# tum-vision/LDSO

Hardware: AMD Instinct MI355X
Metric: GN iters/sec + Mresiduals/sec, 7-KF/2000-pt window (higher is better)
Workload: dtype f32; 1 GPU; C3: 7 KF x 2000 pt x 8 px, 640x480, R=12000, forced GN iterations, synthetic rank-6 marginalisation prior H_M/b_M; arithmetic=f32 residuals / Jacobians / accumulators as the reference, f64 stitch and solve, parallelism=1 GPU

## Files before the change

ldso_amd/csrc/ba_reduce.hip:

```cpp
#include <hip/hip_runtime.h>
#include "ba_host.h"

#include "ba_reduce_body.h"

__global__ __launch_bounds__(256) void k_reduce(BaPtrs B, BaDims D, ResSet S, ChunkStarts chunkStart, int hasL, int GSP, int atomicMode,
                                                int hasPrior, float calibPrior, double l1, double il, int itCheck) {
    static_assert(sizeof(BaPtrs) + sizeof(BaDims) + sizeof(ResSet) + sizeof(ChunkStarts) >= 8 * 64 - 60, "k_reduce: ld_touch_kernarg<8> must stay inside the arguments");
    ld_touch_kernarg<8>();
    reduce_body(B, D, S, chunkStart, hasL, GSP, atomicMode, hasPrior, calibPrior, l1, il, itCheck, (int) blockIdx.x);
}

static __device__ __forceinline__ int g_col(int i, int FS) { return (i < 4) ? (8 * FS + i) : (i - 4); }

static __device__ __forceinline__ double sum_f(const double *PC, int F, int base, int stride, int off, double init = 0.0) {
    double q[LD_MAXF];
#pragma unroll
    for (int x = 0; x < LD_MAXF; x++) q[x] = (x < F) ? PC[(size_t) (base + x * stride) * LD_PAIRC + off] : 0.0;
    double v = init;
#pragma unroll
    for (int x = 0; x < LD_MAXF; x++) if (x < F) v += q[x];
    return v;
}
static __device__ __forceinline__ double sum_pairs(const double *PC, int F, int off) {
    double v = 0;
    for (int p0 = 0; p0 < F * F; p0 += 16) {
        double q[16];
#pragma unroll
        for (int x = 0; x < 16; x++) q[x] = (p0 + x < F * F) ? PC[(size_t) (p0 + x) * LD_PAIRC + off] : 0.0;
#pragma unroll
        for (int x = 0; x < 16; x++) if (p0 + x < F * F) v += q[x];
    }
    return v;
}

static __device__ __forceinline__ double top_entry(const double *PC, int F, int i, int j) {
    if (j < 0) {
        if (i < 4) return sum_pairs(PC, F, 288 + i);
        int f = (i - 4) >> 3, a = (i - 4) & 7;
        double v = sum_f(PC, F, f * F, 1, 272 + a);
        return sum_f(PC, F, f, F, 280 + a, v);
    }
    if (i < 4 && j < 4) return sum_pairs(PC, F, 256 + i * 4 + j);
    if (i < 4 || j < 4) {
        int fi = (i < 4) ? j : i, c = (i < 4) ? i : j;
        int f = (fi - 4) >> 3, a = (fi - 4) & 7;
        double v = sum_f(PC, F, f * F, 1, 192 + a * 4 + c);
        return sum_f(PC, F, f, F, 224 + a * 4 + c, v);
    }
    int f = (i - 4) >> 3, a = (i - 4) & 7, g = (j - 4) >> 3, c = (j - 4) & 7;
    if (f == g) {
        double v = sum_f(PC, F, f * F, 1, a * 8 + c);
        return sum_f(PC, F, f, F, 64 + a * 8 + c, v);
    }
    if (f < g) return PC[(size_t) (f * F + g) * LD_PAIRC + 128 + a * 8 + c] + PC[(size_t) (g * F + f) * LD_PAIRC + 128 + c * 8 + a];
    return PC[(size_t) (g * F + f) * LD_PAIRC + 128 + c * 8 + a] + PC[(size_t) (f * F + g) * LD_PAIRC + 128 + a * 8 + c];
}

__global__ __launch_bounds__(256) void k_gather(BaPtrs B, BaDims D, ResSet S, int hasL, int hasPrior, int GSP, double lambdaIn, int solverMode,
                                                float calibPrior, int mode, double *rbuf) {
    const int F = D.F, n = D.n, FS = D.FS;
    const int N = n * n + n;
    const int e = blockIdx.x * blockDim.x + threadIdx.x;
    double lambda = lambdaIn;
    if (solverMode & LDSO_SOLVER_USE_GN) lambda = 0;
    if (solverMode & LDSO_SOLVER_FIX_LAMBDA) lambda = 1e-5;
    const size_t blk = (size_t) n * n + n;
    double *HA = B.sys, *bA = HA + n * n, *HL = bA + n, *bL = HL + n * n, *Hsc = bL + n, *bsc = Hsc + n * n, *HF = bsc + n, *bF = HF + n * n;
    if (mode == 1 && e >= N && e < N + D.P) {
        int i = e - N;
        double v = 0.0;
        if (i >= D.pBegin && i < D.pEnd) { float c = S.candE[i]; if (c >= 0.0f) v = (double) c + 1.0; }
        rbuf[3 * blk + 8 + i] = v;
    }
    if (e >= N) return;
    const int i = (e < n * n) ? e / n : (e - n * n), j = (e < n * n) ? e % n : -1;
    double prH = 0, prb = 0;
    if (j < 0) prb = (i < 4) ? (double) calibPrior * (double) B.calib->cDeltaF[i] : B.frames[(i - 4) >> 3].prior[(i - 4) & 7] * B.frames[(i - 4) >> 3].delta_prior[(i - 4) & 7];
    else if (i == j) prH = (i < 4) ? (double) calibPrior : B.frames[(i - 4) >> 3].prior[(i - 4) & 7];

    double vA, vL, vS;
    if (mode == 2) {
        vA = rbuf[e]; vL = rbuf[blk + e]; vS = rbuf[2 * blk + e];
    } else {
        vA = top_entry(B.pairC, F, i, j);
        vL = hasL ? top_entry(B.pairC + (size_t) F * F * LD_PAIRC, F, i, j) : 0.0;
        int ci = g_col(i, FS), cj = (j >= 0) ? g_col(j, FS) : (8 * FS + 4);
        int r = min(ci, cj), c = max(ci, cj);
        size_t off = (r / 16 == c / 16) ? ((size_t) ci * GSP + cj) : ((size_t) r * GSP + c);
        float q[LD_SC_SPLITS];
#pragma unroll
        for (int sp = 0; sp < LD_SC_SPLITS; sp++) q[sp] = B.scPart[(size_t) sp * GSP * GSP + off];
        vS = 0;
#pragma unroll
        for (int sp = 0; sp < LD_SC_SPLITS; sp++) vS += (double) q[sp];
    }
    if (mode == 1) { rbuf[e] = vA; rbuf[blk + e] = vL; rbuf[2 * blk + e] = vS; return; }
    if (j >= 0) { HA[e] = vA; HL[e] = vL + prH; Hsc[e] = vS; }
    else { bA[i] = vA; bL[i] = vL + prb; bsc[i] = vS; }
    if (j >= 0) {
        double v = (vL + prH) + (hasPrior ? B.HM[e] : 0.0) + vA;
        if (i == j) v *= (1 + lambda);
        v -= vS * (double) (1.0f / (1 + lambda));
        HF[e] = v;
    } else {
        double s = 0;
        if (hasPrior) {
            s = B.bM[i];
            for (int jj = 0; jj < n; jj++) {
                double dj = (jj < 4) ? (double) B.calib->cDeltaF[jj] : B.frames[(jj - 4) >> 3].delta[(jj - 4) & 7];
                s += B.HM[(size_t) i * n + jj] * dj;
            }
        }
        bF[i] = (vL + prb) + s + vA - vS;
    }
}

hipError_t ba_launch_gather(const BaPtrs &B, const BaDims &D, const ResSet &S, bool hasL, bool hasPrior, int GSP, double lambda,
                            const ldso_settings_t &St, int mode, double *rbuf, hipStream_t st) {
    int N = D.n * D.n + D.n + (mode == 1 ? D.P : 0);
    hipLaunchKernelGGL(k_gather, dim3((N + 255) / 256), dim3(256), 0, st, B, D, S, hasL ? 1 : 0, hasPrior ? 1 : 0, GSP, lambda, St.solverMode,
                       St.initialCalibHessian, mode, rbuf);
    return hipGetLastError();
}

hipError_t ba_launch_reduce(const BaPtrs &B, const BaDims &D, const ResSet &S, const ChunkStarts &chunkStart, bool hasL, int GSP, int atomicMode, bool hasPrior,
                            float calibPrior, double l1, double il, int itCheck, hipStream_t st) {
    const int nb = atomicMode ? reduce_grid(D.F, hasL, D.ks, GSP).total : reduce_pairs(D.F, hasL) + LD_SC_SPLITS;
    const size_t lds = atomicMode ? reduce_atomic_lds_bytes() : (size_t) (SC_SLAB * GSP) * sizeof(float);
    return launch_lds(k_reduce, dim3(nb), dim3(256), lds, st, B, D, S, chunkStart, hasL ? 1 : 0, GSP, atomicMode, hasPrior ? 1 : 0, calibPrior, l1, il, itCheck);
}

__global__ __launch_bounds__(256) void k_marg_update(BaPtrs B, BaDims D, double w) {
    const int n = D.n, e = blockIdx.x * blockDim.x + threadIdx.x;
    const double *HA = B.sys, *bA = HA + n * n, *Hsc = bA + n + (size_t) n * n + n, *bsc = Hsc + n * n;
    if (e < n * n) B.HM[e] += (HA[e] - Hsc[e]) * w;
    else if (e < n * n + n) B.bM[e - n * n] += (bA[e - n * n] - bsc[e - n * n]) * w;
}

hipError_t ba_launch_marg_update(const BaPtrs &B, const BaDims &D, double w, hipStream_t st) {
    const int N = D.n * D.n + D.n;
    hipLaunchKernelGGL(k_marg_update, dim3((N + 255) / 256), dim3(256), 0, st, B, D, w);
    return hipGetLastError();
}

__global__ __launch_bounds__(256) void k_reduce_batch_marg(const BatchItem *__restrict__ items, const MargWin *__restrict__ mw, int nWin) {
    int w = 0;
    for (int i = 1; i < nWin; i++) if ((int) blockIdx.x >= mw[i].redBlock0) w = i;
    const MargWin m = mw[w];
    if (!m.active) return;
    const BatchItem &it = items[w];
    reduce_body(it.B, it.D, it.set[1], it.cs, 0, it.GSP, 0, 0, 0.0f, 1.0, 1.0, -1, (int) blockIdx.x - m.redBlock0);
}

hipError_t ba_launch_reduce_batch_marg(const BatchItem *d_items, const MargWin *d_mw, int nWin, int totalBlocks, int maxGSP, hipStream_t st) {
    if (totalBlocks <= 0) return hipSuccess;
    return launch_lds(k_reduce_batch_marg, dim3(totalBlocks), dim3(256), (size_t) (SC_SLAB * maxGSP) * sizeof(float), st, d_items, d_mw, nWin);
}

__global__ __launch_bounds__(256) void k_marg_gather_update_batch(const BatchItem *__restrict__ items, const MargWin *__restrict__ mw, double w, double *__restrict__ out) {
    const MargWin m = mw[blockIdx.y];
    if (!m.active) return;
    const BatchItem &it = items[blockIdx.y];
    const int F = it.D.F, n = it.D.n, FS = it.D.FS, GSP = it.GSP;
    const int e = blockIdx.x * blockDim.x + threadIdx.x;
    if (e >= n * n + n) return;
    const int i = (e < n * n) ? e / n : (e - n * n), j = (e < n * n) ? e % n : -1;
    const double vA = top_entry(it.B.pairC, F, i, j);
    const int ci = g_col(i, FS), cj = (j >= 0) ? g_col(j, FS) : (8 * FS + 4);
    const int r = min(ci, cj), c = max(ci, cj);
    const size_t off = (r / 16 == c / 16) ? ((size_t) ci * GSP + cj) : ((size_t) r * GSP + c);
    float q[LD_SC_SPLITS];
#pragma unroll
    for (int sp = 0; sp < LD_SC_SPLITS; sp++) q[sp] = it.B.scPart[(size_t) sp * GSP * GSP + off];
    double vS = 0;
#pragma unroll
    for (int sp = 0; sp < LD_SC_SPLITS; sp++) vS += (double) q[sp];
    double *dst = (j >= 0) ? it.B.HM + e : it.B.bM + i;
    double v = it.hasPrior ? *dst : 0.0;
    v += (vA - vS) * w;
    *dst = v;
    out[(size_t) m.outOff + e] = v;
}

hipError_t ba_launch_marg_gather_update_batch(const BatchItem *d_items, const MargWin *d_mw, int nWin, int maxN, double w, double *d_out, hipStream_t st) {
    const int N = maxN * maxN + maxN;
    hipLaunchKernelGGL(k_marg_gather_update_batch, dim3((N + 255) / 256, nWin), dim3(256), 0, st, d_items, d_mw, w, d_out);
    return hipGetLastError();
}

static __device__ __forceinline__ void marg_frame_body(BaPtrs B, BaDims D, int idx, double *W, double *outH, double *outb) {
    const int tid = threadIdx.x, n = D.n, nd = n - 8;
    double *Hs = W, *bs = W + (size_t) n * n;
    __shared__ double sSV[8 * LD_MAXF + 4], sHpi[64], sLU[64], sBLI[(8 * LD_MAXF + 4) * 8];
    __shared__ int sPiv[8];
    auto perm = [&](int i) { const int io = 4 + 8 * idx; return (i < io) ? i : (i < nd) ? i + 8 : io + (i - nd); };
    const DevFrame &fh = B.frames[idx];
    for (int e = tid; e < n * n; e += 256) {
        const int i = e / n, j = e % n;
        double v = B.HM[(size_t) perm(i) * n + perm(j)];
        if (i == j && i >= nd) v += fh.prior[i - nd];
        Hs[e] = v;
    }
    for (int i = tid; i < n; i += 256) bs[i] = B.bM[perm(i)] + ((i >= nd) ? fh.prior[i - nd] * fh.delta_prior[i - nd] : 0.0);
    __syncthreads();
    for (int i = tid; i < n; i += 256) sSV[i] = sqrt(fabs(Hs[(size_t) i * n + i]) + 10.0);
    __syncthreads();
    for (int e = tid; e < n * n; e += 256) { const int i = e / n, j = e % n; Hs[e] = (1.0 / sSV[i]) * Hs[e] * (1.0 / sSV[j]); }
    for (int i = tid; i < n; i += 256) bs[i] = (1.0 / sSV[i]) * bs[i];
    __syncthreads();
    if (tid < 64) { const int r = tid >> 3, c = tid & 7; const double v = Hs[(size_t) (nd + r) * n + nd + c]; sLU[tid] = 0.5 * (v + v); }
    __syncthreads();
    if (tid == 0) {
        for (int k = 0; k < 8; k++) {
            int p = k; double best = fabs(sLU[k * 8 + k]);
            for (int i = k + 1; i < 8; i++) if (fabs(sLU[i * 8 + k]) > best) { best = fabs(sLU[i * 8 + k]); p = i; }
            sPiv[k] = p;
            if (p != k) for (int j = 0; j < 8; j++) { double t = sLU[k * 8 + j]; sLU[k * 8 + j] = sLU[p * 8 + j]; sLU[p * 8 + j] = t; }
            for (int i = k + 1; i < 8; i++) {
                sLU[i * 8 + k] /= sLU[k * 8 + k];
                for (int j = k + 1; j < 8; j++) sLU[i * 8 + j] -= sLU[i * 8 + k] * sLU[k * 8 + j];
            }
        }
    }
    __syncthreads();
    if (tid < 8) {
        double x[8];
        for (int i = 0; i < 8; i++) x[i] = (i == tid) ? 1.0 : 0.0;
        for (int k = 0; k < 8; k++) { const int p = sPiv[k]; if (p != k) { double t = x[k]; x[k] = x[p]; x[p] = t; } }
        for (int i = 0; i < 8; i++) for (int j = 0; j < i; j++) x[i] -= sLU[i * 8 + j] * x[j];
        for (int i = 7; i >= 0; i--) { for (int j = i + 1; j < 8; j++) x[i] -= sLU[i * 8 + j] * x[j]; x[i] /= sLU[i * 8 + i]; }
        for (int i = 0; i < 8; i++) sHpi[i * 8 + tid] = x[i];
    }
    __syncthreads();
    if (tid < 64) sHpi[tid] = 0.5 * (sHpi[tid] + sHpi[tid]);
    __syncthreads();
    for (int e = tid; e < nd * 8; e += 256) {
        const int i = e >> 3, c = e & 7;
        double s_ = 0;
        for (int k = 0; k < 8; k++) s_ += Hs[(size_t) (nd + k) * n + i] * sHpi[k * 8 + c];
        sBLI[e] = s_;
    }
    __syncthreads();
    for (int e = tid; e < nd * (nd + 1); e += 256) {
        const int i = e / (nd + 1), j = e % (nd + 1);
        const double *bl = sBLI + i * 8;
        double s_ = 0;
        if (j < nd) { for (int k = 0; k < 8; k++) s_ += bl[k] * Hs[(size_t) (nd + k) * n + j]; Hs[(size_t) i * n + j] -= s_; }
        else { for (int k = 0; k < 8; k++) s_ += bl[k] * bs[nd + k]; bs[i] -= s_; }
    }
    __syncthreads();
    for (int e = tid; e < nd * nd; e += 256) {
        const int i = e / nd, j = e % nd;
        outH[e] = 0.5 * (sSV[i] * Hs[(size_t) i * n + j] * sSV[j] + sSV[j] * Hs[(size_t) j * n + i] * sSV[i]);
    }
    for (int i = tid; i < nd; i += 256) outb[i] = sSV[i] * bs[i];
}

__global__ __launch_bounds__(256) void k_marg_frame(BaPtrs B, BaDims D, int idx, double *W, double *outH, double *outb) {
    marg_frame_body(B, D, idx, W, outH, outb);
}

__global__ __launch_bounds__(256) void k_marg_frame_batch(const BatchItem *__restrict__ items, const MargWin *__restrict__ mw, double *__restrict__ out) {
    const MargWin m = mw[blockIdx.x];
    if (!m.active) return;
    const BatchItem &it = items[blockIdx.x];
    const int n = it.D.n, nd = n - 8;
    if (!it.hasPrior) {
        for (int e = threadIdx.x; e < n * n; e += 256) it.B.HM[e] = 0.0;
        for (int e = threadIdx.x; e < n; e += 256) it.B.bM[e] = 0.0;
        __syncthreads();
    }
    double *oH = out + m.outOff;
    marg_frame_body(it.B, it.D, m.frameIdx, it.B.sys, oH, oH + (size_t) nd * nd);
}

hipError_t ba_launch_marg_frame_batch(const BatchItem *d_items, int nWin, const MargWin *d_mw, double *d_out, hipStream_t st) {
    hipLaunchKernelGGL(k_marg_frame_batch, dim3(nWin), dim3(256), 0, st, d_items, d_mw, d_out);
    return hipGetLastError();
}

hipError_t ba_launch_marg_frame(const BaPtrs &B, const BaDims &D, int idx, double *work, double *outH, double *outb, hipStream_t st) {
    hipLaunchKernelGGL(k_marg_frame, dim3(1), dim3(256), 0, st, B, D, idx, work, outH, outb);
    return hipGetLastError();
}

__global__ __launch_bounds__(256) void k_acc_init(BaPtrs B, BaDims D, GnInit gi) {
    const int n = D.n, e = blockIdx.x * blockDim.x + threadIdx.x;
    if (e >= n * n + n) return;
    double v = 0.0;
    if (e < n * n && gi.enable == 1) {
        const int i = e / n, j = e % n;
        if (j <= i) {
            if (gi.hasPrior) v = B.HM[e];
            if (i == j) v += (i < 4) ? (double) gi.calibPrior : B.frames[(i - 4) >> 3].prior[(i - 4) & 7];
        }
    }
    B.acc[e] = v;
}

hipError_t ba_launch_acc_init(const BaPtrs &B, const BaDims &D, const GnInit &gi, hipStream_t st) {
    const int N = D.n * D.n + D.n;
    hipLaunchKernelGGL(k_acc_init, dim3((N + 255) / 256), dim3(256), 0, st, B, D, gi);
    return hipGetLastError();
}
```

ldso_amd/csrc/ba_reduce_body.h:

```cpp
#pragma once
#include <hip/hip_runtime.h>
#include "ba_dev.h"

typedef float f32x4 __attribute__((ext_vector_type(4)));
#define SC_SLAB 128
#define PA_SLICES 2
#define PA_UNROLL 24
#define SCT_KS LD_SCT_KS
#define SCT_SLAB 512
#define SC_MAXT 12

__host__ __device__ constexpr int tri13r(int r, int c) { return r * 13 - (r * (r - 1)) / 2 + (c - r); }
__host__ __device__ constexpr size_t reduce_atomic_lds_bytes() { return (size_t) (2 * SCT_SLAB * 16 + SCT_SLAB) * sizeof(float); }

static __device__ __forceinline__ void acc_add(double *p, double v) { __hip_atomic_fetch_add(p, v, __ATOMIC_RELAXED, __HIP_MEMORY_SCOPE_AGENT); }

template <int NT, int W> static __device__ __forceinline__ void schur_wave(const float *sG, int GSP, int cnt, int wcol, int li, int lk, f32x4 *acc);

static __device__ __forceinline__ void reduce_body(const BaPtrs &B, const BaDims &D, const ResSet &S, const ChunkStarts &chunkStart, int hasL, int GSP, int atomicMode,
                                   int hasPrior, float calibPrior, double l1, double il, int itCheck, const int bid) {
    if (LD_ITER_SKIPPED(B, itCheck)) return;
    const int F = D.F, FS = D.FS;
    const int nPairBlocks = reduce_pairs(F, hasL);
    const int tid = threadIdx.x;
    __shared__ double sA[13 * 13];
    __shared__ double sT[2][64];
    const long long t0_ = wall_clock64();
#define RSTAMP(i) do { if (LD_STAMP_ON && tid == 0) B.energyLog[(i)] = (double) (wall_clock64() - t0_); } while (0)

    if (bid < nPairBlocks) {
        const int which = bid / (F * F);
        const int pair = bid % (F * F);
        const int h = pair / F, t = pair % F;
        const float *part = which ? S.topL : S.topA;
        const int c0 = chunkStart.v[h], c1 = chunkStart.v[h + 1];
        if (bid == 0 && c1 > c0) RSTAMP(22);
        __shared__ double sAH[64], sAT[64];
        __shared__ double sPart[PA_SLICES][LD_TOPN];
        if (tid >= 128 && tid < 192) { sAH[tid - 128] = B.adHost[(size_t) (h + t * F) * 64 + (tid - 128)]; }
        if (tid >= 192) { sAT[tid - 192] = B.adTarget[(size_t) (h + t * F) * 64 + (tid - 192)]; }
        const int slice = tid / LD_TOPN, ent = tid % LD_TOPN;
        if (slice < PA_SLICES) {
            double a = 0;
            for (int cb = c0 + slice; cb < c1; cb += PA_SLICES * PA_UNROLL) {
                float q[PA_UNROLL];
#pragma unroll
                for (int u = 0; u < PA_UNROLL; u++) {
                    const int c = cb + u * PA_SLICES, cc = max(min(c, c1 - 1), 0);
                    const float v = part[((unsigned) cc * (unsigned) FS + (unsigned) t) * LD_TOPN + (unsigned) ent];
                    q[u] = (c < c1) ? v : 0.0f;
                }
#pragma unroll
                for (int u = 0; u < PA_UNROLL; u++) a += (double) q[u];
            }
            sPart[slice][ent] = a;
            if (bid == 0 && a != 12345.678) RSTAMP(23);
        }
        __syncthreads();
        if (bid == 0) RSTAMP(20);
        if (tid < LD_TOPN) {
            double a = sPart[0][tid];
#pragma unroll
            for (int sl = 1; sl < PA_SLICES; sl++) a += sPart[sl][tid];
            int r = 0, rem = tid;
            while (rem >= 13 - r) { rem -= 13 - r; r++; }
            int cidx = r + rem;
            sA[r * 13 + cidx] = a;
            sA[cidx * 13 + r] = a;
        }
        __syncthreads();
        double *out = B.pairC + ((size_t) which * F * F + pair) * LD_PAIRC;
        const double *AH = sAH, *AT = sAT;
        if (tid < 64) {
            int i = tid >> 3, j = tid & 7;
            double th = 0, tt = 0;
            for (int m = 0; m < 8; m++) { th += AH[i * 8 + m] * sA[(4 + m) * 13 + 4 + j]; tt += AT[i * 8 + m] * sA[(4 + m) * 13 + 4 + j]; }
            sT[0][tid] = th; sT[1][tid] = tt;
        }
        __syncthreads();
        const int n = D.n;
        double *accT = B.acc, *accb = B.acc + (size_t) n * n;
        const int rh = 4 + 8 * h, rt = 4 + 8 * t;
        if (tid < 64) {
            int i = tid >> 3, j = tid & 7;
            double hh = 0, tt = 0, ht = 0;
            for (int m = 0; m < 8; m++) { hh += sT[0][i * 8 + m] * AH[j * 8 + m]; tt += sT[1][i * 8 + m] * AT[j * 8 + m]; ht += sT[0][i * 8 + m] * AT[j * 8 + m]; }
            if (!atomicMode) { out[tid] = hh; out[64 + tid] = tt; out[128 + tid] = ht; }
            else {
                if (i >= j) { const double dsc = (i == j) ? l1 : 1.0; acc_add(&accT[(size_t) (rh + i) * n + rh + j], hh * dsc); acc_add(&accT[(size_t) (rt + i) * n + rt + j], tt * dsc); }
                if (h > t) acc_add(&accT[(size_t) (rh + i) * n + rt + j], ht);
                else if (h < t) acc_add(&accT[(size_t) (rt + j) * n + rh + i], ht);
            }
        } else if (tid < 64 + 32) {
            int e = tid - 64, i = e >> 2, c = e & 3;
            double hc = 0, tc = 0;
            for (int m = 0; m < 8; m++) { hc += AH[i * 8 + m] * sA[(4 + m) * 13 + c]; tc += AT[i * 8 + m] * sA[(4 + m) * 13 + c]; }
            if (!atomicMode) { out[192 + e] = hc; out[224 + e] = tc; }
            else { acc_add(&accT[(size_t) (rh + i) * n + c], hc); acc_add(&accT[(size_t) (rt + i) * n + c], tc); }
        } else if (tid < 96 + 16) {
            int e = tid - 96;
            if (!atomicMode) out[256 + e] = sA[(e >> 2) * 13 + (e & 3)];
            else if ((e >> 2) >= (e & 3)) acc_add(&accT[(size_t) (e >> 2) * n + (e & 3)], sA[(e >> 2) * 13 + (e & 3)] * (((e >> 2) == (e & 3)) ? l1 : 1.0));
        } else if (tid < 112 + 8) {
            int i = tid - 112;
            double bh = 0, bt = 0;
            for (int m = 0; m < 8; m++) { bh += AH[i * 8 + m] * sA[(4 + m) * 13 + 12]; bt += AT[i * 8 + m] * sA[(4 + m) * 13 + 12]; }
            if (!atomicMode) { out[272 + i] = bh; out[280 + i] = bt; }
            else { acc_add(&accb[rh + i], bh); acc_add(&accb[rt + i], bt); }
        } else if (tid < 120 + 4) {
            int i = tid - 120;
            if (!atomicMode) out[288 + i] = sA[i * 13 + 12];
            else acc_add(&accb[i], sA[i * 13 + 12]);
        }
        if (bid == 0) RSTAMP(21);
        return;
    }

    const int nSplitBase = nPairBlocks;
    const int KS = D.ks;
    if (atomicMode && bid < nSplitBase + reduce_tiles(KS, GSP)) {
        extern __shared__ __attribute__((aligned(16))) float sT_[];
        float *sAc = sT_, *sBc = sAc + SCT_SLAB * 16, *sWc = sBc + SCT_SLAB * 16;
        const int bb = bid - nSplitBase, tile = bb / KS, ks = bb % KS;
        const int nT = GSP / 16, GS = D.GS, n = D.n;
        int ti = 0, rem = tile;
        while (rem >= nT - ti) { rem -= nT - ti; ti++; }
        const int tj = ti + rem;
        const int P0 = D.pBegin, Pn = D.pEnd - D.pBegin, per = ((Pn + KS - 1) / KS + 3) & ~3;
        const int pa = P0 + ks * per, pb = min(P0 + Pn, pa + per);
        const int wave = tid >> 6, lane = tid & 63, li = lane & 15, lk = lane >> 4;
        const int wcol = 8 * FS + 5;
        f32x4 acc = (f32x4){0.f, 0.f, 0.f, 0.f}, acc2 = acc;
        for (int base = pa; base < pb; base += SCT_SLAB) {
            const int cnt = min(SCT_SLAB, pb - base), rows = (cnt + 3) & ~3;
            __syncthreads();
            {
                float4 q[16];
                float wq[2];
#pragma unroll
                for (int u = 0; u < 16; u++) {
                    const int e = tid + u * 256, r = e >> 3, half = (e >> 2) & 1, c4 = e & 3;
                    const int col = (half ? tj : ti) * 16 + c4 * 4;
                    const float4 v = *(const float4 *) (S.G + (unsigned) ((base + min(r, cnt - 1)) * GS + min(col, GS - 4)));
                    const bool in = r < cnt && col < GS;
                    q[u] = make_float4(in ? v.x : 0.f, in ? v.y : 0.f, in ? v.z : 0.f, in ? v.w : 0.f);
                }
#pragma unroll
                for (int u = 0; u < 2; u++) { const int r = tid + u * 256; const float v = S.G[(unsigned) ((base + min(r, cnt - 1)) * GS + wcol)]; wq[u] = (r < cnt) ? v : 0.f; }
#pragma unroll
                for (int u = 0; u < 16; u++) {
                    const int e = tid + u * 256, r = e >> 3, half = (e >> 2) & 1, c4 = e & 3;
                    if (r < rows) *(float4 *) ((half ? sBc : sAc) + r * 16 + c4 * 4) = q[u];
                }
#pragma unroll
                for (int u = 0; u < 2; u++) { const int r = tid + u * 256; if (r < rows) sWc[r] = wq[u]; }
            }
            __syncthreads();
            if (bb == 0) RSTAMP(25);
#pragma unroll 4
            for (int k0 = wave * 4; k0 < rows; k0 += 32) {
                const int k1 = k0 + 16;
                const float a0 = sAc[(k0 + lk) * 16 + li] * sWc[k0 + lk], b0 = sBc[(k0 + lk) * 16 + li];
                const bool in1 = k1 < rows;
                const int k1c = in1 ? k1 : k0;
                const float a1 = in1 ? sAc[(k1c + lk) * 16 + li] * sWc[k1c + lk] : 0.f, b1 = sBc[(k1c + lk) * 16 + li];
                acc = __builtin_amdgcn_mfma_f32_16x16x4f32(a0, b0, acc, 0, 0, 0);
                acc2 = __builtin_amdgcn_mfma_f32_16x16x4f32(a1, b1, acc2, 0, 0, 0);
            }
        }
        __syncthreads();
        if (bb == 0) RSTAMP(26);
        float *sR = sT_;
#pragma unroll
        for (int r = 0; r < 4; r++) sR[wave * 256 + (lk * 4 + r) * 16 + li] = acc[r] + acc2[r];
        __syncthreads();
        {
            const float v = ((sR[tid] + sR[256 + tid]) + sR[512 + tid]) + sR[768 + tid];
            const int rr = ti * 16 + (tid >> 4), cc = tj * 16 + (tid & 15);
            const int F8 = 8 * D.F, FS8 = 8 * FS;
            const int I = (rr < F8) ? 4 + rr : (rr >= FS8 && rr < FS8 + 4) ? rr - FS8 : (rr == FS8 + 4) ? n : -1;
            const int J = (cc < F8) ? 4 + cc : (cc >= FS8 && cc < FS8 + 4) ? cc - FS8 : (cc == FS8 + 4) ? n : -1;
            const bool use = !(ti == tj && rr > cc) && I >= 0 && J >= 0 && I != n;
            if (use) {
                if (J == n) acc_add(&B.acc[(size_t) n * n + I], -(double) v);
                else acc_add(&B.acc[(size_t) max(I, J) * n + min(I, J)], -(double) v * il);
            }
        }
        if (bb == 0) RSTAMP(27);
        return;
    }
    if (atomicMode == 2) return;
    if (atomicMode) {
        const int n = D.n;
        __shared__ double sDelta[8 * LD_MAXF + 4];
        if (tid < n) sDelta[tid] = (tid < 4) ? (double) B.calib->cDeltaF[tid] : B.frames[(tid - 4) >> 3].delta[(tid - 4) & 7];
        double prb = 0, prH = 0, bm = 0;
        if (tid < n) {
            if (tid < 4) { prH = (double) calibPrior; prb = (double) calibPrior * (double) B.calib->cDeltaF[tid]; }
            else { const DevFrame &f = B.frames[(tid - 4) >> 3]; prH = f.prior[(tid - 4) & 7]; prb = prH * f.delta_prior[(tid - 4) & 7]; }
            if (hasPrior) bm = B.bM[tid];
        }
        const int rowT = tid >> 2, quarter = tid & 3;
        constexpr int QW = 16;
        double hq[QW];
        const int per = (n + 3) >> 2, j0 = quarter * per;
        const bool rowOn = hasPrior && rowT < n && 4 * n <= 256;
#pragma unroll
        for (int u = 0; u < QW; u++) hq[u] = (rowOn && u < per && j0 + u < n) ? B.HM[(size_t) rowT * n + j0 + u] : 0.0;
        __syncthreads();
        double part = 0;
#pragma unroll
        for (int u = 0; u < QW; u++) if (u < per && j0 + u < n) part += hq[u] * sDelta[j0 + u];
        part += __shfl_xor(part, 1, 64); part += __shfl_xor(part, 2, 64);
        __shared__ double sHd[8 * LD_MAXF + 4];
        if (quarter == 0 && rowT < n) sHd[rowT] = part;
        __syncthreads();
        if (tid < n) {
            double s_ = 0;
            if (hasPrior) {
                s_ = bm;
                if (4 * n <= 256) s_ += sHd[tid];
                else for (int j0_ = 0; j0_ < n; j0_ += 16) {
                    double q[16];
#pragma unroll
                    for (int u = 0; u < 16; u++) q[u] = (j0_ + u < n) ? B.HM[(size_t) tid * n + j0_ + u] : 0.0;
#pragma unroll
                    for (int u = 0; u < 16; u++) if (j0_ + u < n) s_ += q[u] * sDelta[j0_ + u];
                }
            }
            acc_add(&B.acc[(size_t) n * n + tid], prb + s_);
            const double dterm = prH + (hasPrior ? B.HM[(size_t) tid * n + tid] : 0.0);
            acc_add(&B.acc[(size_t) tid * n + tid], dterm * (l1 - 1.0));
        }
        RSTAMP(28);
        return;
    }

    extern __shared__ __attribute__((aligned(16))) float sG[];
    const int sp = bid - nSplitBase;
    const int wave = tid >> 6, lane = tid & 63;
    const int nT = GSP / 16;
    const int P0 = D.pBegin, Pn = D.pEnd - D.pBegin;
    const int per = (Pn + LD_SC_SPLITS - 1) / LD_SC_SPLITS;
    const int pa = P0 + sp * per, pb = min(P0 + Pn, pa + per);
    const int GS = D.GS;
    const int li = lane & 15, lk = lane >> 4;
    float *Mout = B.scPart + (size_t) sp * GSP * GSP;
    f32x4 acc[SC_MAXT];
#pragma unroll
    for (int q = 0; q < SC_MAXT; q++) acc[q] = (f32x4){0.f, 0.f, 0.f, 0.f};
    for (int base = pa; base < pb; base += SC_SLAB) {
        const int cnt = min(SC_SLAB, pb - base);
        __syncthreads();
        {
            const int g4 = GS >> 2, p4 = GSP >> 2;
            const int rows = (cnt + 3) & ~3;
            for (int e0 = tid; e0 < rows * p4; e0 += 256 * 8) {
                float4 q[8];
#pragma unroll
                for (int u = 0; u < 8; u++) {
                    const int e = e0 + u * 256, r = e / p4, c = e % p4;
                    q[u] = make_float4(0.f, 0.f, 0.f, 0.f);
                    if (e < rows * p4 && r < cnt && c < g4) q[u] = ((const float4 *) (S.G + (size_t) (base + r) * GS))[c];
                }
#pragma unroll
                for (int u = 0; u < 8; u++) { const int e = e0 + u * 256; if (e < rows * p4) ((float4 *) sG)[e] = q[u]; }
            }
        }
        __syncthreads();
        if (sp == 0) RSTAMP(22);
        const int wcol = 8 * FS + 5;
        if (nT == 5) {
            if (wave == 0) schur_wave<5, 0>(sG, GSP, cnt, wcol, li, lk, acc); else if (wave == 1) schur_wave<5, 1>(sG, GSP, cnt, wcol, li, lk, acc);
            else if (wave == 2) schur_wave<5, 2>(sG, GSP, cnt, wcol, li, lk, acc); else schur_wave<5, 3>(sG, GSP, cnt, wcol, li, lk, acc);
        } else {
            if (wave == 0) schur_wave<9, 0>(sG, GSP, cnt, wcol, li, lk, acc); else if (wave == 1) schur_wave<9, 1>(sG, GSP, cnt, wcol, li, lk, acc);
            else if (wave == 2) schur_wave<9, 2>(sG, GSP, cnt, wcol, li, lk, acc); else schur_wave<9, 3>(sG, GSP, cnt, wcol, li, lk, acc);
        }
    }
    if (sp == 0) RSTAMP(23);
    {
        const int n = D.n, F8 = 8 * D.F, FS8 = 8 * FS;
        double *accS = B.acc, *accSb = accS + (size_t) n * n;
        const double *unused_ = nullptr; (void) unused_;
        for (int pass = 0; pass < 1; pass++) {
            int tileIdx = 0;
            for (int ti = 0; ti < nT; ti++)
                for (int tj = ti; tj < nT; tj++, tileIdx++) {
                    if ((tileIdx & 3) != wave) continue;
                    const int q = tileIdx >> 2;
                    f32x4 a4 = acc[0];
#pragma unroll
                    for (int u = 1; u < SC_MAXT; u++) if (u == q) a4 = acc[u];
#pragma unroll
                    for (int r = 0; r < 4; r++) {
                        const int rr = ti * 16 + lk * 4 + r, cc = tj * 16 + li;
                        if (!atomicMode) { Mout[(size_t) rr * GSP + cc] = a4[r]; continue; }
                        if (ti == tj && rr > cc) continue;
                        const int I = (rr < F8) ? 4 + rr : (rr >= FS8 && rr < FS8 + 4) ? rr - FS8 : (rr == FS8 + 4) ? n : -1;
                        const int J = (cc < F8) ? 4 + cc : (cc >= FS8 && cc < FS8 + 4) ? cc - FS8 : (cc == FS8 + 4) ? n : -1;
                        if (I < 0 || J < 0 || I == n) continue;
                        if (J == n) acc_add(&accSb[I], -(double) a4[r]);
                        else acc_add(&accS[(size_t) max(I, J) * n + min(I, J)], -(double) a4[r] * il);
                    }
                }
        }
    }
    if (sp == 0) RSTAMP(24);
}

template <int NT, int W>
static __device__ __forceinline__ void schur_wave(const float *sG, int GSP, int cnt, int wcol, int li, int lk, f32x4 *acc) {
#pragma unroll 2
    for (int k0 = 0; k0 < cnt; k0 += 4) {
        const float *row = sG + (k0 + lk) * GSP;
        float val[NT];
#pragma unroll
        for (int c = 0; c < NT; c++) val[c] = row[c * 16 + li];
        const float w = row[wcol];
        int idx = 0;
#pragma unroll
        for (int ti = 0; ti < NT; ti++)
#pragma unroll
            for (int tj = ti; tj < NT; tj++, idx++)
                if ((idx & 3) == W) acc[idx >> 2] = __builtin_amdgcn_mfma_f32_16x16x4f32(val[ti] * w, val[tj], acc[idx >> 2], 0, 0, 0);
    }
}
```

ldso_amd/csrc/ba_solve.hip:

```cpp
#include <hip/hip_runtime.h>
#include "ba_host.h"

#include "ba_reduce_body.h"
#include "ba_solve_body.h"

__global__ __launch_bounds__(NT) void k_solve(BaPtrs B, BaDims D, ResSet S, ldso_settings_t St, SolveArgs A) {
    solve_body(B, D, S, St, A, (int) gridDim.x, (int) blockIdx.x);
}

__global__ __launch_bounds__(NT) void k_gn_solve(BaPtrs B, BaDims D, ResSet S, ldso_settings_t St, SolveArgs A) {
    static_assert(sizeof(BaPtrs) + sizeof(BaDims) + sizeof(ResSet) + sizeof(ldso_settings_t) + sizeof(SolveArgs) >= 10 * 64 - 60, "k_gn_solve: ld_touch_kernarg<10> must stay inside the arguments");
    if (LD_SOLVE_NB(D.n) == 4) ld_touch_kernarg<10>();
    gn_solve_body<false>(B, D, S, St, A, (int) blockIdx.x);
}

__global__ __launch_bounds__(NT) void k_reduce_solve(BaPtrs B, BaDims D, ResSet S, ldso_settings_t St, SolveArgs A, ChunkStarts chunkStart, int atomicMode,
                                                     float calibPrior, double l1, double il) {
    static_assert(sizeof(BaPtrs) + sizeof(BaDims) + sizeof(ResSet) + sizeof(ldso_settings_t) + sizeof(SolveArgs) + sizeof(ChunkStarts) + 24 >= 12 * 64 - 60, "k_reduce_solve: ld_touch_kernarg<12> must stay inside the arguments");
    ld_touch_kernarg<12>();
    if (blockIdx.x >= LD_FUSED_CTL) {
        const long long tStart_ = LD_STAMP_ON ? wall_clock64() : 0;
        if (LD_ITER_SKIPPED(B, A.itCheck)) return;
        const ReduceGrid rg = reduce_grid(D.F, A.hasL, D.ks, A.GSP);
        const int q = (int) blockIdx.x - LD_FUSED_CTL;
        const int bid = (q < rg.nTile) ? rg.nPair + q : (q < rg.nTile + rg.nPair) ? q - rg.nTile : q;
        reduce_body(B, D, S, chunkStart, A.hasL, A.GSP, atomicMode, A.hasPrior, calibPrior, l1, il, -1, bid);
        __builtin_amdgcn_s_waitcnt(0);
        __syncthreads();
        if (threadIdx.x == 0) {
            const int prev = __hip_atomic_fetch_add(A.waitCtr, 1, __ATOMIC_RELAXED, __HIP_MEMORY_SCOPE_AGENT);
            if (LD_STAMP_ON && prev == A.waitTarget - 1) { B.energyLog[29] = (double) wall_clock64(); B.energyLog[30] = (double) bid; B.energyLog[31] = (double) tStart_; }
        }
        return;
    }
    gn_solve_body<true>(B, D, S, St, A, (int) blockIdx.x);
}

hipError_t ba_launch_solve(const BaPtrs &B, const BaDims &D, const ResSet &S, const ldso_settings_t &St, const SolveArgs &A, hipStream_t st) {
    return launch_lds(k_solve, dim3(solve_roles(A.flags)), dim3(NT), solve_lds_bytes(D.n), st, B, D, S, St, A);
}

hipError_t ba_launch_gn_solve(const BaPtrs &B, const BaDims &D, const ResSet &S, const ldso_settings_t &St, const SolveArgs &A, hipStream_t st) {
    return launch_lds(k_gn_solve, dim3(2), dim3(NT), gn_lds_bytes(D.F, D.n), st, B, D, S, St, A);
}

hipError_t ba_launch_reduce_solve(const BaPtrs &B, const BaDims &D, const ResSet &S, const ldso_settings_t &St, const SolveArgs &A, const ChunkStarts &chunkStart,
                                  int atomicMode, float calibPrior, double l1, double il, hipStream_t st) {
    const ReduceGrid rg = reduce_grid(D.F, A.hasL, D.ks, A.GSP);
    SolveArgs A2 = A;
    A2.waitTarget = rg.total;
    return launch_lds(k_reduce_solve, dim3(rg.total + LD_FUSED_CTL), dim3(NT), std::max(gn_lds_bytes(D.F, D.n), reduce_atomic_lds_bytes()), st,
                      B, D, S, St, A2, chunkStart, atomicMode, calibPrior, l1, il);
}
```

ldso_amd/csrc/ba_solve_batch.hip:

```cpp
#include <hip/hip_runtime.h>
#include "ba_host.h"

#include "ba_reduce_body.h"
#include "ba_solve_body.h"

#define LD_REDB_BLOCKS 4
#define LD_REDB_DENSE_PER_CU 6
static __device__ __forceinline__ void reduce_batch_body(const BatchItem *__restrict__ items, int nWin, int cur, float calibPrior, double l1, double il, int itCheck) {
    int w = 0;
    for (int i = 1; i < nWin; i++) if ((int) blockIdx.x >= items[i].redBlock0) w = i;
    const BatchItem &it = items[w];
    reduce_body(it.B, it.D, it.set[cur], it.cs, 0, it.GSP, 1, it.hasPrior, calibPrior, l1, il, itCheck, (int) blockIdx.x - it.redBlock0);
}
__global__ __launch_bounds__(NT) void k_reduce_batch(const BatchItem *__restrict__ items, int nWin, int cur, float calibPrior, double l1, double il, int itCheck) {
    reduce_batch_body(items, nWin, cur, calibPrior, l1, il, itCheck);
}
__global__ __launch_bounds__(NT, LD_REDB_BLOCKS) void k_reduce_batch_dense(const BatchItem *__restrict__ items, int nWin, int cur, float calibPrior, double l1, double il, int itCheck) {
    reduce_batch_body(items, nWin, cur, calibPrior, l1, il, itCheck);
}

__global__ __launch_bounds__(NT) void k_gn_solve_batch(const BatchItem *__restrict__ items, int cur, ldso_settings_t St, int iteration, double lambda, int logIdx, int itCheck) {
    const BatchItem &it = items[blockIdx.x >> 1];
    SolveArgs A;
    A.iteration = iteration; A.lambda = lambda; A.hasPrior = it.hasPrior; A.GSP = it.GSP; A.logIdx = logIdx; A.itCheck = itCheck;
    gn_solve_body<false>(it.B, it.D, it.set[cur], St, A, (int) (blockIdx.x & 1));
}

__global__ __launch_bounds__(64) void k_batch_begin(const BatchItem *__restrict__ items, int mnumOptIts, int forceAll) {
    const BatchItem &it = items[blockIdx.x];
    it.B.energyLog[threadIdx.x] = 0.0;
    if (threadIdx.x == 0) it.B.scalars[LD_SC_STOP] = (double) (optimize_iteration_cap(it.D.F, mnumOptIts, forceAll) - 1);
}
__global__ __launch_bounds__(NT) void k_solve_batch(const BatchItem *__restrict__ items, ldso_settings_t St, unsigned flags, int phase, int nRoles, double *__restrict__ scalarsOut) {
    const int w = (int) blockIdx.x / nRoles, role = (int) blockIdx.x % nRoles;
    const BatchItem &it = items[w];
    const int stop = (int) it.B.scalars[LD_SC_STOP], applied = stop & 1;
    SolveArgs A;
    A.flags = flags; A.hasPrior = it.hasPrior; A.GSP = it.GSP; A.logIdx = stop + 1 + phase;
    solve_body(it.B, it.D, it.set[applied ^ phase], St, A, nRoles, role);
    if (scalarsOut != nullptr) {
        __syncthreads();
        if (threadIdx.x < 16) scalarsOut[(size_t) it.outSlot * 16 + threadIdx.x] = it.B.scalars[threadIdx.x];
    }
}

hipError_t ba_launch_reduce_batch(const BatchItem *d_items, int nWin, int totalBlocks, int cur, float calibPrior, double l1, double il, hipStream_t st, int itCheck) {
    static int numCU[64] = {0};
    int dev = 0;
    if (hipGetDevice(&dev) != hipSuccess || dev < 0 || dev >= 64) dev = 0;
    if (numCU[dev] == 0) { int cu = 0; if (hipDeviceGetAttribute(&cu, hipDeviceAttributeMultiprocessorCount, dev) != hipSuccess || cu <= 0) cu = 256; numCU[dev] = cu; }
    return launch_lds(totalBlocks >= LD_REDB_DENSE_PER_CU * numCU[dev] ? k_reduce_batch_dense : k_reduce_batch, dim3(totalBlocks), dim3(NT), reduce_atomic_lds_bytes(), st,
                      d_items, nWin, cur, calibPrior, l1, il, itCheck);
}

hipError_t ba_launch_gn_solve_batch(const BatchItem *d_items, int nWin, const BaDims &Dmax, int cur, const ldso_settings_t &St, int iteration, double lambda, hipStream_t st, int logIdx, int itCheck) {
    return launch_lds(k_gn_solve_batch, dim3(2 * nWin), dim3(NT), gn_lds_bytes(Dmax.F, Dmax.n), st, d_items, cur, St, iteration, lambda, logIdx, itCheck);
}

hipError_t ba_launch_batch_begin(const BatchItem *d_items, int nWin, int mnumOptIts, int forceAll, hipStream_t st) {
    hipLaunchKernelGGL(k_batch_begin, dim3(nWin), dim3(64), 0, st, d_items, mnumOptIts, forceAll);
    return hipGetLastError();
}

hipError_t ba_launch_solve_batch(const BatchItem *d_items, int nWin, const BaDims &Dmax, const ldso_settings_t &St, unsigned flags, int phase, double *d_scalarsOut, hipStream_t st) {
    const int nRoles = solve_roles(flags);
    return launch_lds(k_solve_batch, dim3(nRoles * nWin), dim3(NT), solve_lds_bytes(Dmax.n), st, d_items, St, flags, phase, nRoles, d_scalarsOut);
}
```

Before: 29600 GN iters/s.

## Load Schur tile operands directly into registers via buffer loads, bypassing LDS staging

Adds a template variant of reduce_body that, in the single-window and fused reduce-solve paths, reads the A, B and weight columns for each MFMA tile straight from global memory into registers using raw buffer loads with out-of-range masking. This removes the LDS staging slab and its two block barriers per slab, and shrinks the dynamic LDS request so more blocks can be resident per CU. The batched and marginalisation paths keep the staged variant. In exchange, global loads are uncoalesced per-column scalar reads, and a dummy comparison keeps the accumulator live for the timing stamp.

```diff
diff --git a/ldso_amd/csrc/ba_reduce.hip b/ldso_amd/csrc/ba_reduce.hip
--- a/ldso_amd/csrc/ba_reduce.hip
+++ b/ldso_amd/csrc/ba_reduce.hip
@@ -7,7 +7,7 @@
                                                 int hasPrior, float calibPrior, double l1, double il, int itCheck) {
     static_assert(sizeof(BaPtrs) + sizeof(BaDims) + sizeof(ResSet) + sizeof(ChunkStarts) >= 8 * 64 - 60, "k_reduce: ld_touch_kernarg<8> must stay inside the arguments");
     ld_touch_kernarg<8>();
-    reduce_body(B, D, S, chunkStart, hasL, GSP, atomicMode, hasPrior, calibPrior, l1, il, itCheck, (int) blockIdx.x);
+    reduce_body<RT_DIRECT>(B, D, S, chunkStart, hasL, GSP, atomicMode, hasPrior, calibPrior, l1, il, itCheck, (int) blockIdx.x);
 }
 
 static __device__ __forceinline__ int g_col(int i, int FS) { return (i < 4) ? (8 * FS + i) : (i - 4); }
@@ -126,7 +126,7 @@
 hipError_t ba_launch_reduce(const BaPtrs &B, const BaDims &D, const ResSet &S, const ChunkStarts &chunkStart, bool hasL, int GSP, int atomicMode, bool hasPrior,
                             float calibPrior, double l1, double il, int itCheck, hipStream_t st) {
     const int nb = atomicMode ? reduce_grid(D.F, hasL, D.ks, GSP).total : reduce_pairs(D.F, hasL) + LD_SC_SPLITS;
-    const size_t lds = atomicMode ? reduce_atomic_lds_bytes() : (size_t) (SC_SLAB * GSP) * sizeof(float);
+    const size_t lds = atomicMode ? reduce_atomic_lds_bytes(RT_DIRECT) : (size_t) (SC_SLAB * GSP) * sizeof(float);
     return launch_lds(k_reduce, dim3(nb), dim3(256), lds, st, B, D, S, chunkStart, hasL ? 1 : 0, GSP, atomicMode, hasPrior ? 1 : 0, calibPrior, l1, il, itCheck);
 }
 
@@ -149,7 +149,7 @@
     const MargWin m = mw[w];
     if (!m.active) return;
     const BatchItem &it = items[w];
-    reduce_body(it.B, it.D, it.set[1], it.cs, 0, it.GSP, 0, 0, 0.0f, 1.0, 1.0, -1, (int) blockIdx.x - m.redBlock0);
+    reduce_body<RT_STAGED>(it.B, it.D, it.set[1], it.cs, 0, it.GSP, 0, 0, 0.0f, 1.0, 1.0, -1, (int) blockIdx.x - m.redBlock0);
 }
 
 hipError_t ba_launch_reduce_batch_marg(const BatchItem *d_items, const MargWin *d_mw, int nWin, int totalBlocks, int maxGSP, hipStream_t st) {
diff --git a/ldso_amd/csrc/ba_reduce_body.h b/ldso_amd/csrc/ba_reduce_body.h
--- a/ldso_amd/csrc/ba_reduce_body.h
+++ b/ldso_amd/csrc/ba_reduce_body.h
@@ -8,15 +8,25 @@
 #define PA_UNROLL 24
 #define SCT_KS LD_SCT_KS
 #define SCT_SLAB 512
+#define SCT_BATCH 256
 #define SC_MAXT 12
 
+enum ReduceTiles { RT_STAGED, RT_DIRECT };
+
 __host__ __device__ constexpr int tri13r(int r, int c) { return r * 13 - (r * (r - 1)) / 2 + (c - r); }
-__host__ __device__ constexpr size_t reduce_atomic_lds_bytes() { return (size_t) (2 * SCT_SLAB * 16 + SCT_SLAB) * sizeof(float); }
+__host__ __device__ constexpr size_t reduce_atomic_lds_bytes(ReduceTiles tiles) {
+    return (tiles == RT_DIRECT ? (size_t) 4 * 256 : (size_t) (2 * SCT_SLAB * 16 + SCT_SLAB)) * sizeof(float);
+}
 
 static __device__ __forceinline__ void acc_add(double *p, double v) { __hip_atomic_fetch_add(p, v, __ATOMIC_RELAXED, __HIP_MEMORY_SCOPE_AGENT); }
+#define LD_BUFFER_RAW_DWORDS 0x00020000
+static __device__ __forceinline__ float buffer_float(__amdgpu_buffer_rsrc_t rsrc, unsigned byteOffset) {
+    return __builtin_bit_cast(float, __builtin_amdgcn_raw_buffer_load_b32(rsrc, (int) byteOffset, 0, 0));
+}
 
 template <int NT, int W> static __device__ __forceinline__ void schur_wave(const float *sG, int GSP, int cnt, int wcol, int li, int lk, f32x4 *acc);
 
+template <ReduceTiles TILES>
 static __device__ __forceinline__ void reduce_body(const BaPtrs &B, const BaDims &D, const ResSet &S, const ChunkStarts &chunkStart, int hasL, int GSP, int atomicMode,
                                    int hasPrior, float calibPrior, double l1, double il, int itCheck, const int bid) {
     if (LD_ITER_SKIPPED(B, itCheck)) return;
@@ -120,7 +130,6 @@
     const int KS = D.ks;
     if (atomicMode && bid < nSplitBase + reduce_tiles(KS, GSP)) {
         extern __shared__ __attribute__((aligned(16))) float sT_[];
-        float *sAc = sT_, *sBc = sAc + SCT_SLAB * 16, *sWc = sBc + SCT_SLAB * 16;
         const int bb = bid - nSplitBase, tile = bb / KS, ks = bb % KS;
         const int nT = GSP / 16, GS = D.GS, n = D.n;
         int ti = 0, rem = tile;
@@ -131,45 +140,78 @@
         const int wave = tid >> 6, lane = tid & 63, li = lane & 15, lk = lane >> 4;
         const int wcol = 8 * FS + 5;
         f32x4 acc = (f32x4){0.f, 0.f, 0.f, 0.f}, acc2 = acc;
-        for (int base = pa; base < pb; base += SCT_SLAB) {
-            const int cnt = min(SCT_SLAB, pb - base), rows = (cnt + 3) & ~3;
+        if constexpr (TILES == RT_DIRECT) {
+            const int wv = __builtin_amdgcn_readfirstlane(wave);
+            const int colA = ti * 16 + li, colB = tj * 16 + li;
+            constexpr unsigned OUTSIDE = 0x80000000u;
+            const unsigned rowB = 4u * (unsigned) GS, oA = colA < GS ? 4u * (unsigned) colA : OUTSIDE, oB = colB < GS ? 4u * (unsigned) colB : OUTSIDE, oW = 4u * (unsigned) wcol;
+            const unsigned r0 = (unsigned) (4 * wv + lk) * rowB;
+            for (int base = pa; base < pb; base += SCT_BATCH) {
+                const int cnt = min(SCT_BATCH, pb - base), rows = (cnt + 3) & ~3;
+                const __amdgpu_buffer_rsrc_t rowsG = __builtin_amdgcn_make_buffer_rsrc((void *) (S.G + (size_t) base * GS), (short) 0, cnt * (int) rowB, LD_BUFFER_RAW_DWORDS);
+                float aq[16], bq[16], wq[16];
+#pragma unroll
+                for (int s = 0; s < 16; s++) {
+                    const unsigned ro = r0 + (unsigned) (16 * s) * rowB;
+                    aq[s] = buffer_float(rowsG, ro + oA); bq[s] = buffer_float(rowsG, ro + oB); wq[s] = buffer_float(rowsG, ro + oW);
+                }
+#pragma unroll
+                for (int s = 0; s < 16; s++) asm volatile("" : "+v"(aq[s]), "+v"(bq[s]), "+v"(wq[s]));
+                if (bb == 0 && base == pa) RSTAMP(25);
+#pragma unroll
+                for (int j = 0; j < 8; j++) {
+                    const int k0 = 4 * wv + 32 * j;
+                    if (k0 < rows) {
+                        const bool in1 = k0 + 16 < rows;
+                        const float a0 = aq[2 * j] * wq[2 * j], b0 = bq[2 * j];
+                        const float a1 = in1 ? aq[2 * j + 1] * wq[2 * j + 1] : 0.f, b1 = in1 ? bq[2 * j + 1] : bq[2 * j];
+                        acc = __builtin_amdgcn_mfma_f32_16x16x4f32(a0, b0, acc, 0, 0, 0);
+                        acc2 = __builtin_amdgcn_mfma_f32_16x16x4f32(a1, b1, acc2, 0, 0, 0);
+                    }
+                }
+            }
+        } else {
+            float *sAc = sT_, *sBc = sAc + SCT_SLAB * 16, *sWc = sBc + SCT_SLAB * 16;
+            for (int base = pa; base < pb; base += SCT_SLAB) {
+                const int cnt = min(SCT_SLAB, pb - base), rows = (cnt + 3) & ~3;
+                __syncthreads();
+                {
+                    float4 q[16];
+                    float wq[2];
+#pragma unroll
+                    for (int u = 0; u < 16; u++) {
+                        const int e = tid + u * 256, r = e >> 3, half = (e >> 2) & 1, c4 = e & 3;
+                        const int col = (half ? tj : ti) * 16 + c4 * 4;
+                        const float4 v = *(const float4 *) (S.G + (unsigned) ((base + min(r, cnt - 1)) * GS + min(col, GS - 4)));
+                        const bool in = r < cnt && col < GS;
+                        q[u] = make_float4(in ? v.x : 0.f, in ? v.y : 0.f, in ? v.z : 0.f, in ? v.w : 0.f);
+                    }
+#pragma unroll
+                    for (int u = 0; u < 2; u++) { const int r = tid + u * 256; const float v = S.G[(unsigned) ((base + min(r, cnt - 1)) * GS + wcol)]; wq[u] = (r < cnt) ? v : 0.f; }
+#pragma unroll
+                    for (int u = 0; u < 16; u++) {
+                        const int e = tid + u * 256, r = e >> 3, half = (e >> 2) & 1, c4 = e & 3;
+                        if (r < rows) *(float4 *) ((half ? sBc : sAc) + r * 16 + c4 * 4) = q[u];
+                    }
+#pragma unroll
+                    for (int u = 0; u < 2; u++) { const int r = tid + u * 256; if (r < rows) sWc[r] = wq[u]; }
+                }
+                __syncthreads();
+                if (bb == 0) RSTAMP(25);
+#pragma unroll 4
+                for (int k0 = wave * 4; k0 < rows; k0 += 32) {
+                    const int k1 = k0 + 16;
+                    const float a0 = sAc[(k0 + lk) * 16 + li] * sWc[k0 + lk], b0 = sBc[(k0 + lk) * 16 + li];
+                    const bool in1 = k1 < rows;
+                    const int k1c = in1 ? k1 : k0;
+                    const float a1 = in1 ? sAc[(k1c + lk) * 16 + li] * sWc[k1c + lk] : 0.f, b1 = sBc[(k1c + lk) * 16 + li];
+                    acc = __builtin_amdgcn_mfma_f32_16x16x4f32(a0, b0, acc, 0, 0, 0);
+                    acc2 = __builtin_amdgcn_mfma_f32_16x16x4f32(a1, b1, acc2, 0, 0, 0);
+                }
+            }
             __syncthreads();
-            {
-                float4 q[16];
-                float wq[2];
-#pragma unroll
-                for (int u = 0; u < 16; u++) {
-                    const int e = tid + u * 256, r = e >> 3, half = (e >> 2) & 1, c4 = e & 3;
-                    const int col = (half ? tj : ti) * 16 + c4 * 4;
-                    const float4 v = *(const float4 *) (S.G + (unsigned) ((base + min(r, cnt - 1)) * GS + min(col, GS - 4)));
-                    const bool in = r < cnt && col < GS;
-                    q[u] = make_float4(in ? v.x : 0.f, in ? v.y : 0.f, in ? v.z : 0.f, in ? v.w : 0.f);
-                }
-#pragma unroll
-                for (int u = 0; u < 2; u++) { const int r = tid + u * 256; const float v = S.G[(unsigned) ((base + min(r, cnt - 1)) * GS + wcol)]; wq[u] = (r < cnt) ? v : 0.f; }
-#pragma unroll
-                for (int u = 0; u < 16; u++) {
-                    const int e = tid + u * 256, r = e >> 3, half = (e >> 2) & 1, c4 = e & 3;
-                    if (r < rows) *(float4 *) ((half ? sBc : sAc) + r * 16 + c4 * 4) = q[u];
-                }
-#pragma unroll
-                for (int u = 0; u < 2; u++) { const int r = tid + u * 256; if (r < rows) sWc[r] = wq[u]; }
-            }
-            __syncthreads();
-            if (bb == 0) RSTAMP(25);
-#pragma unroll 4
-            for (int k0 = wave * 4; k0 < rows; k0 += 32) {
-                const int k1 = k0 + 16;
-                const float a0 = sAc[(k0 + lk) * 16 + li] * sWc[k0 + lk], b0 = sBc[(k0 + lk) * 16 + li];
-                const bool in1 = k1 < rows;
-                const int k1c = in1 ? k1 : k0;
-                const float a1 = in1 ? sAc[(k1c + lk) * 16 + li] * sWc[k1c + lk] : 0.f, b1 = sBc[(k1c + lk) * 16 + li];
-                acc = __builtin_amdgcn_mfma_f32_16x16x4f32(a0, b0, acc, 0, 0, 0);
-                acc2 = __builtin_amdgcn_mfma_f32_16x16x4f32(a1, b1, acc2, 0, 0, 0);
-            }
-        }
-        __syncthreads();
-        if (bb == 0) RSTAMP(26);
+        }
+        if (bb == 0 && (TILES == RT_STAGED || acc[0] + acc2[0] != 12345.678f)) RSTAMP(26);
         float *sR = sT_;
 #pragma unroll
         for (int r = 0; r < 4; r++) sR[wave * 256 + (lk * 4 + r) * 16 + li] = acc[r] + acc2[r];
diff --git a/ldso_amd/csrc/ba_solve.hip b/ldso_amd/csrc/ba_solve.hip
--- a/ldso_amd/csrc/ba_solve.hip
+++ b/ldso_amd/csrc/ba_solve.hip
@@ -24,7 +24,7 @@
         const ReduceGrid rg = reduce_grid(D.F, A.hasL, D.ks, A.GSP);
         const int q = (int) blockIdx.x - LD_FUSED_CTL;
         const int bid = (q < rg.nTile) ? rg.nPair + q : (q < rg.nTile + rg.nPair) ? q - rg.nTile : q;
-        reduce_body(B, D, S, chunkStart, A.hasL, A.GSP, atomicMode, A.hasPrior, calibPrior, l1, il, -1, bid);
+        reduce_body<RT_DIRECT>(B, D, S, chunkStart, A.hasL, A.GSP, atomicMode, A.hasPrior, calibPrior, l1, il, -1, bid);
         __builtin_amdgcn_s_waitcnt(0);
         __syncthreads();
         if (threadIdx.x == 0) {
@@ -49,6 +49,6 @@
     const ReduceGrid rg = reduce_grid(D.F, A.hasL, D.ks, A.GSP);
     SolveArgs A2 = A;
     A2.waitTarget = rg.total;
-    return launch_lds(k_reduce_solve, dim3(rg.total + LD_FUSED_CTL), dim3(NT), std::max(gn_lds_bytes(D.F, D.n), reduce_atomic_lds_bytes()), st,
+    return launch_lds(k_reduce_solve, dim3(rg.total + LD_FUSED_CTL), dim3(NT), std::max(gn_lds_bytes(D.F, D.n), reduce_atomic_lds_bytes(RT_DIRECT)), st,
                       B, D, S, St, A2, chunkStart, atomicMode, calibPrior, l1, il);
 }
diff --git a/ldso_amd/csrc/ba_solve_batch.hip b/ldso_amd/csrc/ba_solve_batch.hip
--- a/ldso_amd/csrc/ba_solve_batch.hip
+++ b/ldso_amd/csrc/ba_solve_batch.hip
@@ -10,7 +10,7 @@
     int w = 0;
     for (int i = 1; i < nWin; i++) if ((int) blockIdx.x >= items[i].redBlock0) w = i;
     const BatchItem &it = items[w];
-    reduce_body(it.B, it.D, it.set[cur], it.cs, 0, it.GSP, 1, it.hasPrior, calibPrior, l1, il, itCheck, (int) blockIdx.x - it.redBlock0);
+    reduce_body<RT_STAGED>(it.B, it.D, it.set[cur], it.cs, 0, it.GSP, 1, it.hasPrior, calibPrior, l1, il, itCheck, (int) blockIdx.x - it.redBlock0);
 }
 __global__ __launch_bounds__(NT) void k_reduce_batch(const BatchItem *__restrict__ items, int nWin, int cur, float calibPrior, double l1, double il, int itCheck) {
     reduce_batch_body(items, nWin, cur, calibPrior, l1, il, itCheck);
@@ -49,7 +49,7 @@
     int dev = 0;
     if (hipGetDevice(&dev) != hipSuccess || dev < 0 || dev >= 64) dev = 0;
     if (numCU[dev] == 0) { int cu = 0; if (hipDeviceGetAttribute(&cu, hipDeviceAttributeMultiprocessorCount, dev) != hipSuccess || cu <= 0) cu = 256; numCU[dev] = cu; }
-    return launch_lds(totalBlocks >= LD_REDB_DENSE_PER_CU * numCU[dev] ? k_reduce_batch_dense : k_reduce_batch, dim3(totalBlocks), dim3(NT), reduce_atomic_lds_bytes(), st,
+    return launch_lds(totalBlocks >= LD_REDB_DENSE_PER_CU * numCU[dev] ? k_reduce_batch_dense : k_reduce_batch, dim3(totalBlocks), dim3(NT), reduce_atomic_lds_bytes(RT_STAGED), st,
                       d_items, nWin, cur, calibPrior, l1, il, itCheck);
 }
 
```

Result: faster. 31050 GN iters/s, median of 6 (+4.9%).
